# sebadorn/Physically-based-Rendering

Measured on AMD Instinct MI355X. Metric: Msamples/s (paths/s) @1080p fixed seed; 1/2/4/8 MI355X scaling, higher is better.
Workload: dtype f32

## Files before the change

include/pbr_hip_diag.h:

```cpp
#ifndef PBR_HIP_DIAG_H
#define PBR_HIP_DIAG_H

#include "pbr_hip.h"

#ifdef __cplusplus
extern "C" {
#endif

int pbr_diag_math( pbr_ctx* ctx, int op, const float* x, const float* y, int n, float* out );

int pbr_diag_trace( pbr_ctx* ctx, const float* rays, int n, float* out_t, int32_t* out_face, float* out_normal, uint32_t* out_counts );

int pbr_diag_brdf( pbr_ctx* ctx, const float* in, int n, float* out );

int pbr_diag_new_ray( pbr_ctx* ctx, const float* in, int n, float* out );

int pbr_diag_trace_stream( pbr_ctx* ctx, int lds_slots, const float* rays8, uint32_t n, int repeats, float* out2, double* ms_out );

int pbr_diag_calibrate( pbr_ctx* ctx, int mode, uint64_t table_bytes, uint64_t reads, double* ms_out );

int pbr_diag_last_plan( pbr_ctx* ctx, char* name, size_t capacity, int* tuned );

int pbr_diag_bvh_build_info( pbr_ctx* ctx, int* radius );

int pbr_diag_scene_bytes( pbr_ctx* ctx, uint64_t out[3] );

int pbr_diag_refit_info( pbr_ctx* ctx, uint64_t out[8], double* upload_ms, char* why, size_t capacity );

int pbr_diag_last_kernel( pbr_ctx* ctx, char* name, size_t capacity );

int pbr_diag_launch_fit( pbr_ctx* ctx, double* fixed_ms, double* per_frame_ms );

int pbr_diag_set_knob( pbr_ctx* ctx, const char* name, int value );

int pbr_diag_pin_plan( pbr_ctx* ctx, int plan );

int pbr_diag_get_tile_order( pbr_ctx* ctx, int which, uint32_t* order, uint32_t capacity, uint32_t* count, uint32_t band_first[9] );
int pbr_diag_set_tile_order( pbr_ctx* ctx, const uint32_t* order, uint32_t count, const uint32_t* band_first );

int pbr_diag_last_deal( pbr_ctx* ctx, char* name, size_t capacity, int* learnt );
// ... 18 lines not shown
```

physically-based-rendering_amd/__init__.py:

```python
import ctypes
import os

import numpy as np

from . import build as _build
from . import tiles

_HERE = os.path.dirname(os.path.abspath(__file__))

PBR_OK = 0


class Float4(ctypes.Structure):
    _fields_ = [("x", ctypes.c_float), ("y", ctypes.c_float), ("z", ctypes.c_float), ("w", ctypes.c_float)]


class Camera(ctypes.Structure):
    _fields_ = [("eye", Float4), ("w", Float4), ("u", Float4), ("v", Float4),
                ("focusPoint", ctypes.c_int32 * 2), ("lense", ctypes.c_float * 2)]


class DenoiseParams(ctypes.Structure):
    _fields_ = [("passes", ctypes.c_uint32), ("sigma_color", ctypes.c_float), ("sigma_normal", ctypes.c_float),
                ("sigma_world", ctypes.c_float), ("sigma_albedo", ctypes.c_float)]
# ... 110 lines not shown
        ("pbr_mode_built", [ctypes.c_uint32, ctypes.c_uint32]),
        ("pbr_diag_last_kernel", [_vp, ctypes.c_char_p, ctypes.c_size_t]),
        ("pbr_diag_launch_fit", [_vp, ctypes.POINTER(ctypes.c_double), ctypes.POINTER(ctypes.c_double)]),
        ("pbr_diag_set_knob", [_vp, ctypes.c_char_p, ctypes.c_int]),
        ("pbr_diag_get_tile_order", [_vp, ctypes.c_int, _up, ctypes.c_uint32, _up, _up]),
        ("pbr_diag_set_tile_order", [_vp, _up, ctypes.c_uint32, _up]),
        ("pbr_diag_last_deal", [_vp, ctypes.c_char_p, ctypes.c_size_t, ctypes.POINTER(ctypes.c_int)]),
        ("pbr_diag_bvh_build_info", [_vp, ctypes.POINTER(ctypes.c_int)]),
        ("pbr_render_dof", [_vp, ctypes.c_uint32, ctypes.c_uint32, _fp, ctypes.c_float, ctypes.POINTER(Camera)]),
        ("pbr_diag_last_focus_chain", [_vp, ctypes.POINTER(ctypes.c_double)]),
        ("pbr_render_adaptive", [_vp, ctypes.c_uint32, _fp, ctypes.c_float, ctypes.POINTER(Camera), ctypes.POINTER(AdaptiveParams)]),
        ("pbr_read_tile_stats", [_vp, _up, _fp, ctypes.c_uint32, _up]),
        ("pbr_diag_last_adaptive", [_vp, _up, ctypes.POINTER(ctypes.c_uint64), ctypes.POINTER(ctypes.c_double)]),
        ("pbr_update_vertices", [_vp, ctypes.c_void_p, ctypes.c_uint32]),
        ("pbr_read_bvh", [_vp, ctypes.c_void_p, ctypes.c_uint32, _up]),
        ("pbr_diag_refit_info", [_vp, ctypes.POINTER(ctypes.c_uint64), ctypes.POINTER(ctypes.c_double), ctypes.c_char_p, ctypes.c_size_t])):
    if hasattr(hip, _name):
        getattr(hip, _name).argtypes = _args
hip.pbr_diag_tune_budget.argtypes = [_vp, ctypes.POINTER(ctypes.c_uint32)]

host.pbrh_last_error.restype = ctypes.c_char_p
host.pbrh_cfg_set.argtypes = [ctypes.c_char_p, ctypes.c_char_p]
host.pbrh_cfg_get.argtypes = [ctypes.c_char_p, ctypes.c_char_p, ctypes.c_int]
host.pbrh_cfg_load.argtypes = [ctypes.c_char_p]
host.pbrh_scene_load_obj.argtypes = [ctypes.c_char_p, ctypes.c_char_p]
host.pbrh_scene_load_obj.restype = _vp
host.pbrh_scene_generate.argtypes = [ctypes.c_char_p, ctypes.c_uint32, ctypes.c_uint32]
host.pbrh_scene_generate.restype = _vp
host.pbrh_scene_destroy.argtypes = [_vp]
host.pbrh_scene_destroy.restype = None
host.pbrh_scene_desc.argtypes = [_vp, ctypes.POINTER(SceneDesc)]
# ... 359 lines not shown
    def last_trace(self):
        ms, n = ctypes.c_double(), ctypes.c_uint32()
        self._check(hip.pbr_diag_last_trace(self._ctx, ctypes.byref(ms), ctypes.byref(n)))
        return float(ms.value), int(n.value)

    def last_focus_chain_ms(self):
        ms = ctypes.c_double()
        self._check(hip.pbr_diag_last_focus_chain(self._ctx, ctypes.byref(ms)))
        return float(ms.value)

    def last_plan(self):
        name, tuned = ctypes.create_string_buffer(48), ctypes.c_int(-1)
        self._check(hip.pbr_diag_last_plan(self._ctx, name, 48, ctypes.byref(tuned)))
        return name.value.decode(), int(tuned.value)

    def scene_bytes(self):
        out = (ctypes.c_uint64 * 3)()
        self._check(hip.pbr_diag_scene_bytes(self._ctx, out))
        return {"nodes": int(out[0]), "walk_streams": int(out[1]), "faces": int(out[2])}

    def last_kernel(self):
        name = ctypes.create_string_buffer(96)
        self._check(hip.pbr_diag_last_kernel(self._ctx, name, 96))
        return name.value.decode()

    def launch_fit(self):
        a, b = ctypes.c_double(), ctypes.c_double()
        if hip.pbr_diag_launch_fit(self._ctx, ctypes.byref(a), ctypes.byref(b)) != PBR_OK:
            return None
        return float(a.value), float(b.value)
# ... 125 lines not shown
```

physically-based-rendering_amd/csrc/pbr_hip.hip:

```cpp
#include <hip/hip_runtime.h>

#include <cmath>
#include <cstdarg>
#include <cstdio>
#include <cstdlib>
#include <chrono>
#include <cstring>
#include <string>
#include <algorithm>
#include <vector>

#include "pbr_hip.h"
#include "pbr_hip_diag.h"
#include "pt_aux.hpp"
#include "pt_adaptive.hpp"
#include "pt_instances.hpp"
#include "bvh_build.hpp"
#include "pt_denoise.hpp"
#include "pt_scene_pack.hpp"
#include "pt_tuner.hpp"
#include "pt_deal.hpp"
#include "pt_adaptive_host.hpp"
#include "pt_refit_host.hpp"
#include "pt_refit.hpp"
// ... 438 lines not shown
	return PBR_OK;
}

int sceneParams( pbr_ctx* ctx, DevParams* P, uint32_t* hotAvail = nullptr ) {
	std::memset( P, 0, sizeof( *P ) );
	uint32_t hot = 0;
	const int walk = applyWalk( ctx, P, &hot );

	if( hotAvail != nullptr ) {
		*hotAvail = hot;
	}

	P->parkEighths = 4;
	P->tris = ctx->dTris;
	P->faceN = ctx->dFaceN;
	P->mats = ctx->dMats;
	P->lights = ctx->dLights;
	P->guard = ctx->dGuard;
	P->numNodes = (int) ctx->numNodes;
	P->numLights = (int) ctx->numLights;
	return walk;
}

void setCamera( DevParams* P, const pbr_camera* cam, int w, int h, float pxDim ) {
	const float* src[4] = { &cam->eye.x, &cam->w.x, &cam->u.x, &cam->v.x };
	float* dst[4] = { P->eye, P->cw, P->cu, P->cv };

	for( int i = 0; i < 4; i++ ) {
		for( int k = 0; k < 3; k++ ) {
			dst[i][k] = src[i][k];
// ... 741 lines not shown

	if( ctx->configured ) {
		PBR_TRY( packConfiguredWalk( ctx, ctx->cfg, &tree, &walk ) );
	}

	HIP_TRY( ctx, hipSetDevice( ctx->device ) );
	freeScene( ctx );

	auto toDevice = [ctx]( float4** dst, const std::vector<Quad>& src ) {
		HIP_TRY( ctx, hipMalloc( (void**) dst, sizeof( Quad ) * src.size() ) );
		HIP_TRY( ctx, hipMemcpy( *dst, src.data(), sizeof( Quad ) * src.size(), hipMemcpyHostToDevice ) );
		return PBR_OK;
	};

	PBR_TRY( toDevice( &ctx->dNodes, packed.nodes.storage ) );
	PBR_TRY( toDevice( &ctx->dTris, packed.tris ) );

	if( !packed.triPN.empty() ) {
		PBR_TRY( toDevice( &ctx->dTriPN, packed.triPN ) );
	}

	PBR_TRY( toDevice( &ctx->dMats, packed.mats ) );
	PBR_TRY( toDevice( &ctx->dLights, packed.lights ) );
	ctx->nodeBytes = sizeof( Quad ) * packed.nodes.storage.size();
	ctx->triBytes = sizeof( Quad ) * packed.tris.size();

	if( s->num_faces > 0 && ctx->knobs.faceNormals != 0 ) {
		HIP_TRY( ctx, hipMalloc( (void**) &ctx->dFaceN, sizeof( float4 ) * s->num_faces ) );
		DevParams P;
		std::memset( &P, 0, sizeof( P ) );
		P.tris = ctx->dTris;
		hipLaunchKernelGGL( ptk::prepareFaceNormals, dim3( ( s->num_faces + 255 ) / 256 ), dim3( 256 ), 0, ctx->stream, P, ctx->dFaceN, (int) s->num_faces );
		HIP_TRY( ctx, hipGetLastError() );
	}

	ctx->refitBytes = 0;

	if( refit.nested ) {
		auto keep = [ctx]( void** dst, const void* src, size_t bytes ) {
			HIP_TRY( ctx, hipMalloc( dst, std::max<size_t>( bytes, 16 ) ) );

			if( src != nullptr && bytes > 0 ) {
				HIP_TRY( ctx, hipMemcpy( *dst, src, bytes, hipMemcpyHostToDevice ) );
			}

			ctx->refitBytes += bytes;
			return PBR_OK;
		};
// ... 53 lines not shown
	}
	if( ctx->configured && ctx->cfg.phong_tessellation > 0.0f ) {
		return fail( ctx, PBR_ESTATE, "pbr_update_vertices while Phong tessellation is configured: tight boxes of the flat triangles would clip the patches" );
	}

	HIP_TRY( ctx, hipSetDevice( ctx->device ) );
	const auto uploadStart = std::chrono::steady_clock::now();
	HIP_TRY( ctx, hipMemcpy( ctx->dVertices, vertices, sizeof( pbr_float4 ) * num_vertices, hipMemcpyHostToDevice ) );
	ctx->lastRefitUploadMs = std::chrono::duration<double, std::milli>( std::chrono::steady_clock::now() - uploadStart ).count();

	const uint32_t F = ctx->numFaces;
	HIP_TRY( ctx, hipEventRecord( ctx->evStart, ctx->stream ) );
	hipLaunchKernelGGL( ptr::refitFaces, dim3( ( F + 255 ) / 256 ), dim3( 256 ), 0, ctx->stream, ctx->dFacesV, ctx->dVertices, ctx->dTris, (int) F );
	HIP_TRY( ctx, hipGetLastError() );

	if( ctx->dFaceN != nullptr ) {
		DevParams P;
		std::memset( &P, 0, sizeof( P ) );
		P.tris = ctx->dTris;
		hipLaunchKernelGGL( ptk::prepareFaceNormals, dim3( ( F + 255 ) / 256 ), dim3( 256 ), 0, ctx->stream, P, ctx->dFaceN, (int) F );
		HIP_TRY( ctx, hipGetLastError() );
	}

	hipLaunchKernelGGL( ptr::refitSubtrees, dim3( ctx->refitGroups ), dim3( REFIT_SUBTREE ), 0, ctx->stream, ctx->dRefitSlots, ctx->dRefitInfo,
	                    ctx->dRefitHeights, ctx->dRefitRecordOf, ctx->dFacesV, ctx->dVertices, ctx->dNodes, ctx->dRootBox );
	HIP_TRY( ctx, hipGetLastError() );

	if( ctx->refitLevels > 0 ) {
		hipLaunchKernelGGL( ptr::refitTop, dim3( 1 ), dim3( REFIT_TOP_THREADS ), 0, ctx->stream, ctx->dRefitTop, ctx->dRefitLevelFirst, (int) ctx->refitLevels,
		                    ctx->dRefitInfo, ctx->dRefitRecordOf, ctx->dNodes, ctx->dRootBox );
		HIP_TRY( ctx, hipGetLastError() );
	}

	HIP_TRY( ctx, hipEventRecord( ctx->evStop, ctx->stream ) );
	HIP_TRY( ctx, hipStreamSynchronize( ctx->stream ) );
	float ms = 0.0f;
// ... 980 lines not shown
	*radius = ctx->lastBvhRadius;
	return PBR_OK;
}

int pbr_diag_scene_bytes( pbr_ctx* ctx, uint64_t out[3] ) {
	if( ctx == nullptr || out == nullptr || !ctx->hasScene ) {
		return fail( ctx, PBR_ESTATE, "diag_scene_bytes: no scene" );
	}

	out[0] = ctx->nodeBytes;
	out[1] = ctx->walkBytes;
	out[2] = ctx->triBytes;
	return PBR_OK;
}

int pbr_diag_refit_info( pbr_ctx* ctx, uint64_t out[8], double* upload_ms, char* why, size_t capacity ) {
	if( ctx == nullptr || out == nullptr || !ctx->hasScene ) {
		return fail( ctx, PBR_ESTATE, "diag_refit_info: no scene" );
	}

	out[0] = ctx->refit.nested ? 1 : 0;
	out[1] = ctx->refit.subtreeCap;
	out[2] = ctx->refitGroups;
	out[3] = ctx->refitSubtrees;
	out[4] = ctx->refitTopNodes;
	out[5] = ctx->refitLevels;
	out[6] = ctx->refitBytes;
	out[7] = ctx->refitUpdates;

	if( upload_ms != nullptr ) {
// ... 179 lines not shown
```

physically-based-rendering_amd/csrc/pt_aux.hpp:

```cpp
#pragma once

#include "pt_kernel.hpp"
#include "pt_diag.hpp"

namespace ptk {

__global__ __launch_bounds__( 256 ) void foldFrames( const DevParams P, const float4* src, float4* dst ) {
	const unsigned slot = blockIdx.x * blockDim.x + threadIdx.x;

	if( slot <= (unsigned) PT_HEADS ) {
		P.workCounter[slot * PT_BAND_STRIDE] = 0u;
	}

	if( slot >= P.frameStride ) {
		return;
	}

	float4 acc = src[slot];

	for( int k = 0; k < P.nFrames; k++ ) {
		const float4 fc = P.frameBuf[frameBufIndex( P, slot, (unsigned) k )];
		const unsigned n = (unsigned) ( P.firstCount + k );
		const float w = P.useExplicitWeight ? P.explicitWeight : ( (float) n / (float) ( n + 1u ) );
		acc.x = fc.x + ( acc.x - fc.x ) * w;
// ... 21 lines not shown
	if( ( threadIdx.x & 63u ) == 0u ) {
		cost[tile] = v;
	}
}

__global__ void prepareFaceNormals( DevParams P, float4* faceN, int numFaces ) {
	const int face = (int) ( blockIdx.x * blockDim.x + threadIdx.x );

	if( face >= numFaces ) {
		return;
	}

	int material;
	const f3 n = faceNormal<false>( P, face, &material );
	faceN[face] = make_float4( n.x, n.y, n.z, __int_as_float( material ) );
}


__global__ void untile( const float4* tiles, float4* rows, int width, int height, int tilesX, int tileWorld, int tileRank ) {
	const int x = (int) ( blockIdx.x * blockDim.x + threadIdx.x );
	const int y = (int) ( blockIdx.y * blockDim.y + threadIdx.y );

	if( x >= width || y >= height ) {
		return;
	}

	const int tileGlobal = ( y >> 3 ) * tilesX + ( x >> 3 );
	float4 v = make_float4( 0.0f, 0.0f, 0.0f, 0.0f );

	const int position = dealPositionOfTile( tileGlobal, tilesX, tileWorld );
// ... 173 lines not shown
```

physically-based-rendering_amd/csrc/pt_dual.hpp:

```cpp
#ifdef PT_NODE_PHASE_ASM

#define PT_DUAL_SLAB( n0a, n0b, n0c, n0d, n1a, n1b, oxy, ozz, ixy, izz ) \
		"v_pk_add_f32 v[54:55], v[" n0a ":" n0b "], " oxy " neg_lo:[0,1] neg_hi:[0,1]\n" \
		"v_pk_add_f32 v[56:57], v[" n0c ":" n0d "], " oxy " neg_lo:[0,1] neg_hi:[0,1]\n" \
		"v_pk_add_f32 v[58:59], v[" n1a ":" n1b "], " ozz " neg_lo:[0,1] neg_hi:[0,1]\n" \
		"v_pk_mul_f32 v[54:55], " ixy ", v[54:55]\n" \
		"v_pk_mul_f32 v[56:57], " ixy ", v[56:57]\n" \
		"v_pk_mul_f32 v[58:59], " izz ", v[58:59]\n" \
		"v_min_f32 v60, v54, v56\n" \
		"v_min_f32 v61, v55, v57\n" \
		"v_min_f32 v62, v58, v59\n" \
		"v_max3_f32 v60, v60, v61, v62\n" \
		"v_max_f32 v61, v54, v56\n" \
		"v_max_f32 v63, v58, v59\n" \
		"v_max_f32 v62, v55, v57\n" \
		"v_min3_f32 v61, v61, v62, v63\n"
#define PT_DUAL_FETCH( walk, cur, n0, n1lo, n1hi, flag, skip ) \
		"s_mov_b64 exec, " walk "\n" \
		"s_cbranch_execz " skip "9f\n" \
		"v_cmp_gt_i32 vcc, %[numHotBytes], " cur "\n" \
		"s_and_saveexec_b64 s[94:95], vcc\n" \
		"s_cselect_b32 s82, 1, 0\n" \
		"ds_read_b128 v[" n0 "], " cur "\n" \
		"ds_read_b128 v[" n1lo ":" n1hi "], " cur " offset:16\n" \
// ... 282 lines not shown
			if( ( shadeA || shadeB ) && ( nShade >= P.phShade || !busy ) ) {
				const bool useB = !shadeA;
				const int which = useB ? 1 : 0;
				PixelState st;
				loadCold( P, which, st );
				st.ray.origin = useB ? B.ray.origin : A.ray.origin;
				st.ray.dir = useB ? B.ray.dir : A.ray.dir;
				st.dbgNodes += useB ? B.nodes : A.nodes;
				st.dbgTris += useB ? B.tris : A.tris;
				Hit hit;
				hit.t = useB ? B.t : A.t;
				hit.face = useB ? B.face : A.face;
				hit.normal = mk3( 0.0f, 0.0f, 0.0f );
				bool more = true;

				if( shadeStep<BRDF, SHADOW, LIGHTS, false, true, true>( P, lds, st, cnt, hit ) ) {
					finishPixel( P, st );

					if( cnt.nodes > 0x40000000u || cnt.tris > 0x40000000u ) {
						flushCounters( P, cnt );
					}

					unsigned frame = 0;
					const unsigned slot = nextSlot( P, work, (unsigned) P.nFrames, frame );

					if( slot != PT_NO_WORK ) {
						beginPixel( P, st, slot, cnt, frame );
					}
					else {
						more = false;
					}
// ... 20 lines not shown
```

physically-based-rendering_amd/csrc/pt_kernel.hpp:

```cpp
#pragma once

#include <hip/hip_runtime.h>

#include "pt_math.hpp"

#ifdef PBR_GUARD
#define PBR_GUARD_PATH 1
#define PBR_GUARD_TRAV 1
#endif

#ifdef PBR_LAB_HOOKS
#include "pt_lab_hooks.hpp"
#else
#define PT_LAB_TRAVERSE_BEGIN
#define PT_LAB_NODE_ITERATION
#define PT_LAB_LEAF_PHASE
#define PT_LAB_TRAVERSE_END( P, anyhit )
#define PT_LAB_WAVE_BEGIN
#define PT_LAB_WAVE_DRY
#define PT_LAB_WAVE_END_LOCKSTEP( P )
#define PT_LAB_WAVE_END_PHASED( P )
#define PT_LAB_PHASED_BEGIN
#define PT_LAB_PHASED_STAT( what )
#define PT_LAB_PHASED_NODE_BEGIN( mode )
// ... 76 lines not shown
	int numHot;
	int numHotBytes;
	int firstRef;
	int walkScheme;
	const int* walkTable;
	int slotBase;
	int nFrames, firstCount;
	int useExplicitWeight;
	float explicitWeight;
	float pxDim, antiAliasing;
	float sky[3];
	const float4* faceN;
	const float* chain;
	unsigned chainSlotStride, chainFrameStride;
	unsigned chainFocusAt;
};

#define PT_DEAL_SHIFT 5

__host__ __device__ inline int dealPositionOfTile( int tileGlobal, int tilesX, int world ) {
	if( world <= 1 ) {
		return tileGlobal;
	}

	const int ty = tileGlobal / tilesX;
	const int tx = tileGlobal - ty * tilesX;
	return ty * tilesX + ( tx + PT_DEAL_SHIFT * ty ) % tilesX;
}

__host__ __device__ inline int tileAtDealPosition( int position, int tilesX, int world ) {
// ... 32 lines not shown
PT_DEV f3 ld3( const float* p ) { return mk3( p[0], p[1], p[2] ); }

PT_DEV float rnd( float& seed ) {
	seed += 1.0f;
	return fract( sin1( seed ) * 43758.5453123f );
}

PT_DEV float fresnel( float u, float c ) {
	const float v = 1.0f - u;
	return c + ( 1.0f - c ) * v * v * v * v * v;
}

struct TangentFrame {
	f3 n, u, v;
	bool valid;
};

PT_DEV void tangentFrame( f3 n, f3* u, f3* v ) {
	*u = normalize( cross( yzx( n ), n ) );
	*v = normalize( cross( n, *u ) );
}

PT_DEV bool sameBits( f3 a, f3 b ) {
	return __float_as_int( a.x ) == __float_as_int( b.x ) && __float_as_int( a.y ) == __float_as_int( b.y ) && __float_as_int( a.z ) == __float_as_int( b.z );
}

PT_DEV f3 jitterUV( f3 nl, f3 u, f3 v, float phi, float sina, float cosa ) {
	float sp, cp;
	sincos( phi, &sp, &cp );
	const f3 w = normalize( u * cp + v * sp );
	return normalize( w * sina + nl * cosa );
}

PT_DEV f3 jitter( f3 nl, float phi, float sina, float cosa ) {
	f3 u, v;
	tangentFrame( nl, &u, &v );
	return jitterUV( nl, u, v, phi, sina, cosa );
}

// ... 3 lines not shown
	const float4 b = P.mats[index * 4 + 1];
	Material m;
	m.d = a.x; m.Ni = a.y; m.p2 = a.z; m.p3 = a.w;
	m.Rs = b.x; m.Rd = b.y;
	m.colours = P.mats + index * 4 + 2;
	m.Kd = m.Ks = mk3( 0.0f, 0.0f, 0.0f );

	if( !LATE ) {
		const float4 kd = m.colours[0];
		const float4 ks = m.colours[1];
		m.Kd = mk3( kd.x, kd.y, kd.z );
		m.Ks = mk3( ks.x, ks.y, ks.z );
	}

	return m;
}

template<bool LATE = true>
PT_DEV MaterialColours materialColours( const Material& m ) {
	MaterialColours c;

	if( LATE ) {
		const float4 kd = m.colours[0];
		const float4 ks = m.colours[1];
		c.Kd = mk3( kd.x, kd.y, kd.z );
		c.Ks = mk3( ks.x, ks.y, ks.z );
	}
	else {
		c.Kd = m.Kd;
		c.Ks = m.Ks;
// ... 857 lines not shown
PT_DEV f3 faceNormal( const DevParams& P, int face, int* material ) {
	if( STORED && !PT_ARITH_NATIVE && P.faceN != nullptr ) {
		const float4 r = P.faceN[face];
		*material = __float_as_int( r.w );
		return mk3( r.x, r.y, r.z );
	}

	const float4 r0 = P.tris[face * 3 + 0];
	const float4 r1 = P.tris[face * 3 + 1];
	const float4 r2 = P.tris[face * 3 + 2];
	*material = __float_as_int( r2.y );
	return normalize( cross( mk3( r0.w, r1.x, r1.y ), mk3( r1.z, r1.w, r2.x ) ) );
}



PT_DEV Ray initRay( const DevParams& P, int px, int py, float& seed, float tFocus, float tObject ) {
	const f3 cu = ld3( P.cu );
	const f3 cv = ld3( P.cv );
	const float fx = 2.0f * (float) px;
	const float fy = 2.0f * (float) py;

	f3 inner = ld3( P.camA );
	inner = inner + cu * fx;
	inner = inner + cv;
	inner = inner - ld3( P.cvH );
	inner = inner + cv * fy;

	const float s = P.halfPx;
	const f3 initial = ld3( P.cw ) + inner * s;
// ... 41 lines not shown
	return ( x == 0.0f ) ? 0.0f : div1( r, x * x );
}

PT_DEV float schA( float w, float p ) {
	const float p2 = p * p;
	const float w2 = w * w;
	const float x = p2 - p2 * w2 + w2;
	return ( x == 0.0f ) ? 0.0f : sqrt1( div1( p, x ) );
}

PT_DEV float schG( float v, float r ) {
	const float x = r - r * v + v;
	return ( x == 0.0f ) ? 0.0f : div1( v, x );
}

PT_DEV float brdfSchlick( const Material& mtl, f3 outDir, f3 inDir, f3 normal, float* u, float* pdf, const TangentFrame* frame = nullptr ) {
	const f3 vOutV = -outDir;
	f3 un;

	if( frame != nullptr && frame->valid && sameBits( frame->n, normal ) ) {
		un = frame->u;
	}
	else {
		un = normalize( cross( yzx( normal ), normal ) );
	}

	const f3 h = normalize( vOutV + inDir );
	const float t = dot( h, normal );
	const float vIn = dot( inDir, normal );
	const float vOut = dot( vOutV, normal );
	const f3 hp = normalize( cross( cross( h, normal ), normal ) );
	const float w = dot( un, hp );

	*u = dot( h, vOutV );
	*pdf = div1( t, (float) ( (double) 4.0f * M_PI_D * (double) dot( vOutV, h ) ) );
// ... 7 lines not shown
	const float lam = (float) ( (double) a * M_1_PI_D );
	float ani = 0.0f;

	if( !( b == 0.0f || d == 0.0f ) ) {
		const float gp = schG( vOut, r ) * schG( vIn, r );
		const float obstructed = gp * schZ( t, r ) * schA( w, p );
		const float reemission = 1.0f - gp;
		ani = div1( b, d ) * ( obstructed + reemission );
	}

	const float fres = ( vIn == 0.0f ) ? 0.0f : div1( c, vIn );

	return lam + ani + fres;
}

PT_DEV f3 newRaySchlick( f3 dir, f3 normal, const Material& mtl, float& seed, TangentFrame* frame = nullptr ) {
	const float rough = mtl.p3;
	const float iso = mtl.p2;

	if( rough == 0.0f ) {
		return reflect( dir, normal );
	}

	const float a = rnd( seed );
	float b = rnd( seed );
	const float iso2 = iso * iso;
	const float alpha = acos1( sqrt1( div1( a, rough - a * rough + a ) ) );
	float edge, base;
	int mode;

// ... 7 lines not shown
	base = (float) ( M_PI_2_D * (double) sqrt1( div1( iso2 * b2, 1.0f - b2 + b2 * iso2 ) ) );

	float phi = base;

	if( mode == 1 ) { phi = (float) ( M_PI_D - (double) base ); }
	else if( mode == 2 ) { phi = (float) ( M_PI_D + (double) base ); }
	else if( mode == 3 ) { phi = (float) ( (double) 2.0f * M_PI_D - (double) base ); }

	if( iso < 1.0f ) {
		phi = (float) ( (double) phi + M_PI_2_D );
	}

	float sa, ca;
	sincos( alpha, &sa, &ca );
	f3 fu, fv;
	tangentFrame( normal, &fu, &fv );

	if( frame != nullptr ) {
		frame->n = normal;
		frame->u = fu;
		frame->v = fv;
		frame->valid = true;
	}

	const f3 H = jitterUV( normal, fu, fv, phi, sa, ca );
	f3 out = reflect( dir, H );

	if( dot( out, normal ) <= 0.0f ) {
		out = jitterUV( normal, fu, fv, PI_X2 * rnd( seed ), sqrt1( a ), sqrt1( 1.0f - a ) );
	}

	return out;
}



template<bool CALLS = false>
PT_DEV void brdfSA(
	const Material& mtl, f3 outDir, f3 inDir, f3 normal,
	float* brdfSpec, float* brdfDiff, float* dotHK1, float* pdf, const TangentFrame* frame = nullptr
) {
	const float nu = mtl.p2, nv = mtl.p3;
	f3 un, vn;

	if( frame != nullptr && frame->valid && sameBits( frame->n, normal ) ) {
		un = frame->u;
		vn = frame->v;
	}
	else {
		tangentFrame( normal, &un, &vn );
	}

	const f3 k1 = inDir;
	const f3 k2 = -outDir;
	const f3 h = normalize( k1 + k2 );

	const float dotHU = dot( h, un );
	const float dotHV = dot( h, vn );
	const float dotHN = dot( h, normal );
	const float dotNK1 = dot( normal, k1 );
	const float dotNK2 = dot( normal, k2 );
	const float hk1 = dot( h, k1 );
	*dotHK1 = hk1;

	float ps_e = nu * dotHU * dotHU + nv * dotHV * dotHV;
	ps_e = ( dotHN == 1.0f ) ? 0.0f : div1( ps_e, 1.0f - dotHN * dotHN );
	const float ps0 = (float) ( (double) ( sqrt1( ( nu + 1.0f ) * ( nv + 1.0f ) ) * 0.125f ) * M_1_PI_D );
	const float ps1_num = powSelect<CALLS>( dotHN, ps_e );
	const float ps1 = div1( ps1_num, hk1 * fmax1( dotNK1, dotNK2 ) );

	float pd = mtl.Rd * 0.38750768752f;
	const float a = 1.0f - dotNK1 * 0.5f;
	const float b = 1.0f - dotNK2 * 0.5f;
	pd *= 1.0f - a * a * a * a * a;
	pd *= 1.0f - b * b * b * b * b;

	*brdfSpec = ps0 * ps1;
	*brdfDiff = pd;
	*pdf = div1( ps0 * ps1_num, hk1 );
}

template<bool CALLS = false>
PT_DEV f3 newRaySA( f3 dir, f3 rayNormal, const Material& mtl, float& seed, TangentFrame* frame = nullptr ) {
	const float nu = mtl.p2, nv = mtl.p3;
	float a = rnd( seed );
	const float b = rnd( seed );
	float phi_flip = (float) M_PI_D;
	float phi_flipf = 1.0f;
	float aMax = 1.0f;

	if( a < 0.25f ) {
		aMax = 0.25f;
		phi_flip = 0.0f;
	}
	else if( a < 0.5f ) {
		aMax = 0.5f;
		phi_flipf = -1.0f;
	}
	else if( a < 0.75f ) {
		aMax = 0.75f;
	}
	else {
		phi_flip = (float) ( (double) 2.0f * M_PI_D );
		phi_flipf = -1.0f;
	}

	a = 1.0f - 4.0f * ( aMax - a );

	const float phi = atan1( sqrt1( div1( nu + 1.0f, nv + 1.0f ) ) * tan1( (float) ( M_PI_2_D * (double) a ) ) );
	const float phi_full = phi_flip + phi_flipf * phi;

	float sinphi, cosphi;
	sincos( phi, &sinphi, &cosphi );
	const float theta_e = div1( 1.0f, nu * cosphi * cosphi + nv * sinphi * sinphi + 1.0f );
	const float theta = acos1( powSelect<CALLS>( 1.0f - b, theta_e ) );

	const f3 normal = ( mtl.d < 1.0f || dot( rayNormal, -dir ) >= 0.0f ) ? rayNormal : -rayNormal;

	float st, ct;
	sincos( theta, &st, &ct );
	f3 u, v;
	tangentFrame( normal, &u, &v );

	if( frame != nullptr ) {
		frame->n = normal;
		frame->u = u;
		frame->v = v;
		frame->valid = true;
	}

	const f3 h = jitterUV( normal, u, v, phi_full, st, ct );
	const f3 spec = reflect( dir, h );
	const f3 diff = jitterUV( normal, u, v, PI_X2 * rnd( seed ), sqrt1( b ), sqrt1( 1.0f - b ) );

	return ( dot( spec, normal ) <= 0.0f ) ? diff : spec;
}

PT_DEV f3 refract( f3 dir, f3 normal, const Material& mtl, float& seed ) {
	const bool into = ( dot( normal, -dir ) > 0.0f );
	const f3 nl = into ? normal : -normal;
	const float m1 = into ? NI_AIR : mtl.Ni;
	const float m2 = into ? mtl.Ni : NI_AIR;
	const float m = div1( m1, m2 );
// ... 5 lines not shown
	}

	const float sqrtCosT = sqrt1( 1.0f - sinT2 );
	const float r0 = div1( m1 - m2, m1 + m2 );
	const float c = ( m1 > m2 ) ? sqrtCosT : cosI;
	const float reflectance = fresnel( c, r0 * r0 );

	if( reflectance < rnd( seed ) ) {
		const float k = m * cosI - sqrtCosT;
		return dir * m + nl * k;
	}

	return reflect( dir, nl );
}

template<int BRDF, bool CALLS = false>
PT_DEV f3 newRayDir( f3 dir, f3 normal, const Material& mtl, float& seed, bool& addDepth, TangentFrame* frame = nullptr ) {
	bool doTransRefr = false;

	if( mtl.d < 1.0f ) {
		doTransRefr = ( mtl.d <= rnd( seed ) );
	}

	addDepth = addDepth || doTransRefr;

	if( doTransRefr ) {
		return refract( dir, normal, mtl, seed );
	}

	return ( BRDF == 0 ) ? newRaySchlick( dir, normal, mtl, seed, frame ) : newRaySA<CALLS>( dir, normal, mtl, seed, frame );
}

template<int BRDF, bool CALLS = false, bool LATE = true>
PT_DEV f3 throughput( const Material& mtl, f3 outDir, f3 inDir, f3 normal, const TangentFrame* frame = nullptr ) {
	const float d = mtl.d;

	if( BRDF == 0 ) {
		float u, pdf;
		float brdf = brdfSchlick( mtl, outDir, inDir, normal, &u, &pdf, frame );
		brdf *= fmax1( dot( normal, inDir ), 0.0f );
		brdf = div1( brdf, pdf );

		const MaterialColours mc = materialColours<LATE>( mtl );
		const f3 f4 = mk3( fresnel( u, mc.Ks.x ), fresnel( u, mc.Ks.y ), fresnel( u, mc.Ks.z ) );
		const f3 k = mk3( f4.x * brdf * d + ( 1.0f - d ), f4.y * brdf * d + ( 1.0f - d ), f4.z * brdf * d + ( 1.0f - d ) );
		return mc.Kd * k;
	}

	float spec, diff, dotHK1, pdf;
	brdfSA<CALLS>( mtl, outDir, inDir, normal, &spec, &diff, &dotHK1, &pdf, frame );
	spec = div1( spec, pdf );
	diff = div1( diff, pdf );

	const float fr = fresnel( dotHK1, mtl.Rs );
	const MaterialColours mc = materialColours<LATE>( mtl );
	const f3 brdf_s = ( mc.Ks * spec ) * fr;
	const f3 brdf_d = ( mc.Kd * diff ) * ( 1.0f - mtl.Rs );
	f3 bc = brdf_s + brdf_d;
	bc = mk3( bc.x * d + ( 1.0f - d ), bc.y * d + ( 1.0f - d ), bc.z * d + ( 1.0f - d ) );
	const float maxRGB = max_cl( 1.0f, max_cl( bc.x, max_cl( bc.y, bc.z ) ) );
	bc = mk3( div1( bc.x, maxRGB ), div1( bc.y, maxRGB ), div1( bc.z, maxRGB ) );

	return mk3( clamp01( bc.x ), clamp01( bc.y ), clamp01( bc.z ) );
}

template<int BRDF, bool CALLS = false, bool LATE = true>
PT_DEV bool shadowContribution(
	const Material& mtl, f3 outDir, f3 lightDir, f3 normal, f3 color, f3 lightRgb, f3* add, const TangentFrame* frame = nullptr
) {
	const float d = mtl.d;

	if( BRDF == 0 ) {
		float u, pdf;
		float brdf = brdfSchlick( mtl, outDir, lightDir, normal, &u, &pdf, frame );

		if( !( __builtin_fabsf( pdf ) > 0.00001f ) ) {
			return false;
		}

		brdf *= fmax1( dot( normal, lightDir ), 0.0f );
		brdf = div1( brdf, pdf );

		const MaterialColours mc = materialColours<LATE>( mtl );
		const f3 f4 = mk3( fresnel( u, mc.Ks.x ), fresnel( u, mc.Ks.y ), fresnel( u, mc.Ks.z ) );
		const f3 k = mk3( f4.x * brdf * d + ( 1.0f - d ), f4.y * brdf * d + ( 1.0f - d ), f4.z * brdf * d + ( 1.0f - d ) );
		*add = ( ( color * lightRgb ) * mc.Kd ) * k;
		return true;
	}

	float spec, diff, dotHK1, pdf;
	brdfSA<CALLS>( mtl, outDir, lightDir, normal, &spec, &diff, &dotHK1, &pdf, frame );

	if( !( __builtin_fabsf( pdf ) > 0.00001f ) ) {
		return false;
	}

	spec = div1( spec, pdf );
	diff = div1( diff, pdf );

	const float fr = fresnel( dotHK1, mtl.Rs );
	const MaterialColours mc = materialColours<LATE>( mtl );
	const f3 brdf_s = ( mc.Ks * spec ) * fr;
	const f3 brdf_d = ( mc.Kd * diff ) * ( 1.0f - mtl.Rs );
	f3 bc = brdf_s + brdf_d;
	bc = mk3( bc.x * d + ( 1.0f - d ), bc.y * d + ( 1.0f - d ), bc.z * d + ( 1.0f - d ) );
	const float maxRGB = max_cl( 1.0f, max_cl( bc.x, max_cl( bc.y, bc.z ) ) );
// ... 108 lines not shown
	st.depthAdded = 0;
	float tFocus, tObject;
	focusInputs( P, slot, frame, &tFocus, &tObject );
	int px, py;
	pixelOfSlot( P, slot, &px, &py );
	st.ray = initRay( P, px, py, st.seed, tFocus, tObject );
	cnt.paths++;
}

PT_DEV void finishPixel( const DevParams& P, const PixelState& st ) {
	if( P.imgDbg != nullptr && st.frame == P.nFrames ) {
		P.imgDbg[st.slot] = make_float4( (float) st.dbgTris / 1082.0f, (float) st.dbgNodes / 1265.0f, 0.0f, 0.0f );
	}
}

template<int BRDF, bool SHADOW, bool LIGHTS, bool PHONG = false, bool EAGER = false, bool CALLS = !EAGER, bool FACEN = false, bool LATE = true>
PT_DEV bool shadeStep( const DevParams& P, const float4* lds, PixelState& st, LaneCounters& cnt, const Hit hit ) {
	Ray& ray = st.ray;
	f3& color = st.color;
	f3& finalColor = st.finalColor;
	unsigned& secondaryPaths = st.secondaryPaths;
	float& seed = st.seed;
	int& depth = st.depth;
	int& depthAdded = st.depthAdded;
	unsigned& dbgTris = st.dbgTris;
	unsigned& totHits = cnt.hits;

	st.focus = ( st.sample + depth == 0 ) ? hit.t : st.focus;

		bool pathDone = false;
		f3 light = mk3( -1.0f, -1.0f, -1.0f );

		if( hit.t == inff() ) {
			if( LIGHTS && hit.face < 0 ) {
				const float4 rgb = P.lights[( -( hit.face + 1 ) ) * 3 + 1];
				light = mk3( rgb.x, rgb.y, rgb.z );
			}
			else {
				light = ld3( P.sky );
			}

			pathDone = true;
		}
		else {
			int mtlIndex;
			f3 normal = faceNormal<FACEN>( P, hit.face, &mtlIndex );

			if( PHONG ) {
				normal = hit.normal;
			}
			const Material mtl = loadMaterial<LATE>( P, mtlIndex );
			totHits++;

			bool addDepth;

			if( BRDF == 1 ) {
				addDepth = ( fmax1( mtl.p2, mtl.p3 ) >= 50.0f );
			}
			else {
				addDepth = ( mtl.p3 < rnd( seed ) );
			}
// ... 24 lines not shown
						lh.face = 0;
						unsigned unusedNodes = 0;
						traverse<true, LIGHTS, true, PHONG, EAGER>( P, lds, lightRay, lh, unusedNodes, dbgTris );
						lightDir = lightRay.dir;

						if( lh.t >= tLight ) {
							const float4 rgb = P.lights[1];
							lightRgb = mk3( rgb.x, rgb.y, rgb.z );
							lit = ( lightRgb.x >= 0.0f );
						}
					}
				}

				TangentFrame frame;
				frame.valid = false;
				const f3 newDir = newRayDir<BRDF, CALLS>( ray.dir, normal, mtl, seed, addDepth, &frame );

				if( dot( normal, -ray.dir ) <= 0.0f ) {
					normal = -normal;
				}

				if( SHADOW && LIGHTS ) {
					if( lit ) {
						f3 add;

						if( shadowContribution<BRDF, CALLS, LATE>( mtl, ray.dir, lightDir, normal, color, lightRgb, &add, &frame ) ) {
							finalColor = finalColor + add;
							secondaryPaths += 1;
						}
					}
				}

				color = color * throughput<BRDF, CALLS, LATE>( mtl, ray.dir, newDir, normal, &frame );

				depthAdded += ( addDepth && depthAdded < P.maxAddedDepth ) ? 1 : 0;

				const float maxValColor = fmax1( color.x, fmax1( color.y, color.z ) );
				bool terminate = false;

				if( depth > 2 + depthAdded ) {
					terminate = ( maxValColor < rnd( seed ) );
				}

				if( terminate ) {
					pathDone = true;
				}
				else {
					ray.origin = hitPoint;
// ... 401 lines not shown
```

physically-based-rendering_amd/csrc/pt_scene_pack.hpp:

```cpp
#pragma once

#include <algorithm>
#include <cmath>
#include <cstdarg>
#include <cstddef>
#include <cstdint>
#include <cstdio>
#include <cstring>
#include <string>
#include <utility>
#include <vector>

#include "pbr_hip.h"

struct Quad {
	float x, y, z, w;
};
static_assert( sizeof( Quad ) == 16, "a Quad is a float4 on the device" );

constexpr uint32_t kLdsStageBytes = 160 * 1024 - 256;

constexpr size_t kRefLimit = (size_t) 1 << 31;

struct SceneTree {
// ... 488 lines not shown
		}
	}

	const uint32_t lightSlots = ( s->num_lights > 0 ) ? s->num_lights : 1;
	out->lights.assign( (size_t) lightSlots * 3, Quad { 0.0f, 0.0f, 0.0f, 0.0f } );

	for( uint32_t i = 0; i < s->num_lights; i++ ) {
		const pbr_light& l = s->lights[i];
		out->lights[(size_t) i * 3 + 0] = Quad { l.pos.x, l.pos.y, l.pos.z, l.pos.w };
		out->lights[(size_t) i * 3 + 1] = Quad { l.rgb.x, l.rgb.y, l.rgb.z, l.rgb.w };
		out->lights[(size_t) i * 3 + 2] = Quad { l.data.x, l.data.y, l.data.z, l.data.w };
	}

	return PBR_OK;
}
```

Before: 2242.

## Precompute per-face tangent frames and per-material BRDF terms on device

Adds a scene-load and refit pass that stores, for each face, its normal, material index, tangent frame and the tangent frame of the flipped normal, appended after the triangle data. The shading path loads these records instead of rebuilding the frame at every hit. Per-material Ashikhmin-Shirley constants (ps0 and the phi scale) are also packed into the material table so the sqrt/div work per bounce goes away. The cost is extra memory traffic per hit (up to three more float4 loads) and a larger triangle buffer, with a fallback to on-the-fly computation when a stored frame is flagged non-bitwise-identical.

```diff
diff --git a/include/pbr_hip_diag.h b/include/pbr_hip_diag.h
--- a/include/pbr_hip_diag.h
+++ b/include/pbr_hip_diag.h
@@ -24,6 +24,8 @@
 int pbr_diag_bvh_build_info( pbr_ctx* ctx, int* radius );
 
 int pbr_diag_scene_bytes( pbr_ctx* ctx, uint64_t out[3] );
+
+int pbr_diag_face_frames( pbr_ctx* ctx, float* records, float* per_hit );
 
 int pbr_diag_refit_info( pbr_ctx* ctx, uint64_t out[8], double* upload_ms, char* why, size_t capacity );
 
diff --git a/physically-based-rendering_amd/__init__.py b/physically-based-rendering_amd/__init__.py
--- a/physically-based-rendering_amd/__init__.py
+++ b/physically-based-rendering_amd/__init__.py
@@ -148,7 +148,8 @@
         ("pbr_diag_last_adaptive", [_vp, _up, ctypes.POINTER(ctypes.c_uint64), ctypes.POINTER(ctypes.c_double)]),
         ("pbr_update_vertices", [_vp, ctypes.c_void_p, ctypes.c_uint32]),
         ("pbr_read_bvh", [_vp, ctypes.c_void_p, ctypes.c_uint32, _up]),
-        ("pbr_diag_refit_info", [_vp, ctypes.POINTER(ctypes.c_uint64), ctypes.POINTER(ctypes.c_double), ctypes.c_char_p, ctypes.c_size_t])):
+        ("pbr_diag_refit_info", [_vp, ctypes.POINTER(ctypes.c_uint64), ctypes.POINTER(ctypes.c_double), ctypes.c_char_p, ctypes.c_size_t]),
+        ("pbr_diag_face_frames", [_vp, _fp, _fp])):
     if hasattr(hip, _name):
         getattr(hip, _name).argtypes = _args
 hip.pbr_diag_tune_budget.argtypes = [_vp, ctypes.POINTER(ctypes.c_uint32)]
@@ -538,6 +539,12 @@
         self._check(hip.pbr_diag_last_plan(self._ctx, name, 48, ctypes.byref(tuned)))
         return name.value.decode(), int(tuned.value)
 
+    def diag_face_frames(self, num_faces):
+        records = np.empty((num_faces, 16), np.float32)
+        per_hit = np.empty((num_faces, 16), np.float32)
+        self._check(hip.pbr_diag_face_frames(self._ctx, _as_fp(records), _as_fp(per_hit)))
+        return records.view(np.uint32), per_hit.view(np.uint32)
+
     def scene_bytes(self):
         out = (ctypes.c_uint64 * 3)()
         self._check(hip.pbr_diag_scene_bytes(self._ctx, out))
diff --git a/physically-based-rendering_amd/csrc/pbr_hip.hip b/physically-based-rendering_amd/csrc/pbr_hip.hip
--- a/physically-based-rendering_amd/csrc/pbr_hip.hip
+++ b/physically-based-rendering_amd/csrc/pbr_hip.hip
@@ -476,6 +476,7 @@
 	P->parkEighths = 4;
 	P->tris = ctx->dTris;
 	P->faceN = ctx->dFaceN;
+	P->frameFirst = (int) frameFirstQuad( ctx->numFaces );
 	P->mats = ctx->dMats;
 	P->lights = ctx->dLights;
 	P->guard = ctx->dGuard;
@@ -1247,24 +1248,32 @@
 	};
 
 	PBR_TRY( toDevice( &ctx->dNodes, packed.nodes.storage ) );
-	PBR_TRY( toDevice( &ctx->dTris, packed.tris ) );
+	HIP_TRY( ctx, hipMalloc( (void**) &ctx->dTris, sizeof( Quad ) * faceAllocationQuads( s->num_faces ) ) );
+	HIP_TRY( ctx, hipMemset( ctx->dTris, 0, sizeof( Quad ) * faceAllocationQuads( s->num_faces ) ) );
+	HIP_TRY( ctx, hipMemcpy( ctx->dTris, packed.tris.data(), sizeof( Quad ) * packed.tris.size(), hipMemcpyHostToDevice ) );
 
 	if( !packed.triPN.empty() ) {
 		PBR_TRY( toDevice( &ctx->dTriPN, packed.triPN ) );
 	}
 
+	packMaterialTerms( s, &packed.mats );
 	PBR_TRY( toDevice( &ctx->dMats, packed.mats ) );
 	PBR_TRY( toDevice( &ctx->dLights, packed.lights ) );
 	ctx->nodeBytes = sizeof( Quad ) * packed.nodes.storage.size();
-	ctx->triBytes = sizeof( Quad ) * packed.tris.size();
-
-	if( s->num_faces > 0 && ctx->knobs.faceNormals != 0 ) {
-		HIP_TRY( ctx, hipMalloc( (void**) &ctx->dFaceN, sizeof( float4 ) * s->num_faces ) );
+	ctx->triBytes = sizeof( Quad ) * faceAllocationQuads( s->num_faces );
+
+	{
 		DevParams P;
 		std::memset( &P, 0, sizeof( P ) );
 		P.tris = ctx->dTris;
-		hipLaunchKernelGGL( ptk::prepareFaceNormals, dim3( ( s->num_faces + 255 ) / 256 ), dim3( 256 ), 0, ctx->stream, P, ctx->dFaceN, (int) s->num_faces );
+		hipLaunchKernelGGL( ptk::prepareFaceFrames, dim3( ( s->num_faces + 255 ) / 256 ), dim3( 256 ), 0, ctx->stream, P, ctx->dTris + frameFirstQuad( s->num_faces ), (int) s->num_faces );
 		HIP_TRY( ctx, hipGetLastError() );
+
+		if( ctx->knobs.faceNormals != 0 ) {
+			HIP_TRY( ctx, hipMalloc( (void**) &ctx->dFaceN, sizeof( float4 ) * s->num_faces ) );
+			hipLaunchKernelGGL( ptk::prepareFaceNormals, dim3( ( s->num_faces + 255 ) / 256 ), dim3( 256 ), 0, ctx->stream, P, ctx->dFaceN, (int) s->num_faces );
+			HIP_TRY( ctx, hipGetLastError() );
+		}
 	}
 
 	ctx->refitBytes = 0;
@@ -1348,12 +1357,17 @@
 	hipLaunchKernelGGL( ptr::refitFaces, dim3( ( F + 255 ) / 256 ), dim3( 256 ), 0, ctx->stream, ctx->dFacesV, ctx->dVertices, ctx->dTris, (int) F );
 	HIP_TRY( ctx, hipGetLastError() );
 
-	if( ctx->dFaceN != nullptr ) {
+	{
 		DevParams P;
 		std::memset( &P, 0, sizeof( P ) );
 		P.tris = ctx->dTris;
-		hipLaunchKernelGGL( ptk::prepareFaceNormals, dim3( ( F + 255 ) / 256 ), dim3( 256 ), 0, ctx->stream, P, ctx->dFaceN, (int) F );
+		hipLaunchKernelGGL( ptk::prepareFaceFrames, dim3( ( F + 255 ) / 256 ), dim3( 256 ), 0, ctx->stream, P, ctx->dTris + frameFirstQuad( F ), (int) F );
 		HIP_TRY( ctx, hipGetLastError() );
+
+		if( ctx->dFaceN != nullptr ) {
+			hipLaunchKernelGGL( ptk::prepareFaceNormals, dim3( ( F + 255 ) / 256 ), dim3( 256 ), 0, ctx->stream, P, ctx->dFaceN, (int) F );
+			HIP_TRY( ctx, hipGetLastError() );
+		}
 	}
 
 	hipLaunchKernelGGL( ptr::refitSubtrees, dim3( ctx->refitGroups ), dim3( REFIT_SUBTREE ), 0, ctx->stream, ctx->dRefitSlots, ctx->dRefitInfo,
@@ -2364,6 +2378,40 @@
 	return PBR_OK;
 }
 
+int pbr_diag_face_frames( pbr_ctx* ctx, float* records, float* per_hit ) {
+	if( ctx == nullptr || records == nullptr || per_hit == nullptr ) {
+		return fail( ctx, PBR_EINVAL, "diag_face_frames: null argument" );
+	}
+	if( !ctx->hasScene ) {
+		return fail( ctx, PBR_ESTATE, "diag_face_frames: no scene" );
+	}
+
+	const uint32_t F = ctx->numFaces;
+	const size_t bytes = sizeof( float ) * 16 * (size_t) F;
+	float* dOut = nullptr;
+	HIP_TRY( ctx, hipSetDevice( ctx->device ) );
+	HIP_TRY( ctx, hipMalloc( (void**) &dOut, bytes ) );
+	DevParams P;
+	std::memset( &P, 0, sizeof( P ) );
+	P.tris = ctx->dTris;
+	hipLaunchKernelGGL( ptk::faceFramesPerHit, dim3( ( F + 255 ) / 256 ), dim3( 256 ), 0, ctx->stream, P, dOut, (int) F );
+	hipError_t err = hipGetLastError();
+
+	if( err == hipSuccess ) {
+		err = hipStreamSynchronize( ctx->stream );
+	}
+	if( err == hipSuccess ) {
+		err = hipMemcpy( per_hit, dOut, bytes, hipMemcpyDeviceToHost );
+	}
+	if( err == hipSuccess ) {
+		err = hipMemcpy( records, ctx->dTris + frameFirstQuad( F ), bytes, hipMemcpyDeviceToHost );
+	}
+
+	(void) hipFree( dOut );
+	HIP_TRY( ctx, err );
+	return PBR_OK;
+}
+
 int pbr_diag_refit_info( pbr_ctx* ctx, uint64_t out[8], double* upload_ms, char* why, size_t capacity ) {
 	if( ctx == nullptr || out == nullptr || !ctx->hasScene ) {
 		return fail( ctx, PBR_ESTATE, "diag_refit_info: no scene" );
diff --git a/physically-based-rendering_amd/csrc/pt_aux.hpp b/physically-based-rendering_amd/csrc/pt_aux.hpp
--- a/physically-based-rendering_amd/csrc/pt_aux.hpp
+++ b/physically-based-rendering_amd/csrc/pt_aux.hpp
@@ -59,6 +59,49 @@
 	int material;
 	const f3 n = faceNormal<false>( P, face, &material );
 	faceN[face] = make_float4( n.x, n.y, n.z, __int_as_float( material ) );
+}
+
+__global__ void prepareFaceFrames( DevParams P, float4* frames, int numFaces ) {
+	const int face = (int) ( blockIdx.x * blockDim.x + threadIdx.x );
+
+	if( face >= numFaces ) {
+		return;
+	}
+
+	int material;
+	const f3 n = faceNormal<false>( P, face, &material );
+	f3 u, v, ub, vb;
+	tangentFrame( n, &u, &v );
+	tangentFrame( -n, &ub, &vb );
+	const float sum = ( ( n.x + n.y + n.z ) + ( u.x + u.y + u.z ) ) + ( ( v.x + v.y + v.z ) + ( vb.x + vb.y + vb.z ) );
+	const bool finite = ( __builtin_fabsf( sum ) < inff() );
+	const int flags = ( finite && sameBits( u, ub ) ) ? 0 : 1;
+	float4* rec = frames + (size_t) face * PT_FRAME_QUADS;
+	rec[0] = make_float4( n.x, n.y, n.z, __int_as_float( material ) );
+	rec[1] = make_float4( u.x, u.y, u.z, __int_as_float( flags ) );
+	rec[2] = make_float4( v.x, v.y, v.z, 0.0f );
+	rec[3] = make_float4( vb.x, vb.y, vb.z, 0.0f );
+}
+
+__global__ void faceFramesPerHit( DevParams P, float* out, int numFaces ) {
+	const int face = (int) ( blockIdx.x * blockDim.x + threadIdx.x );
+
+	if( face >= numFaces ) {
+		return;
+	}
+
+	int material;
+	const f3 n = faceNormal<false>( P, face, &material );
+	f3 u, v, ub, vb;
+	tangentFrame( n, &u, &v );
+	tangentFrame( -n, &ub, &vb );
+	float* o = out + (size_t) face * 16;
+	o[0] = n.x; o[1] = n.y; o[2] = n.z;
+	o[3] = u.x; o[4] = u.y; o[5] = u.z;
+	o[6] = v.x; o[7] = v.y; o[8] = v.z;
+	o[9] = ub.x; o[10] = ub.y; o[11] = ub.z;
+	o[12] = vb.x; o[13] = vb.y; o[14] = vb.z;
+	o[15] = __int_as_float( material );
 }
 
 
diff --git a/physically-based-rendering_amd/csrc/pt_dual.hpp b/physically-based-rendering_amd/csrc/pt_dual.hpp
--- a/physically-based-rendering_amd/csrc/pt_dual.hpp
+++ b/physically-based-rendering_amd/csrc/pt_dual.hpp
@@ -320,7 +320,9 @@
 				hit.normal = mk3( 0.0f, 0.0f, 0.0f );
 				bool more = true;
 
-				if( shadeStep<BRDF, SHADOW, LIGHTS, false, true, true>( P, lds, st, cnt, hit ) ) {
+				constexpr bool FRAMES = !( PT_WALK_MODE == 1 && BRDF == 1 && SHADOW );
+
+				if( shadeStep<BRDF, SHADOW, LIGHTS, false, true, true, false, true, FRAMES>( P, lds, st, cnt, hit ) ) {
 					finishPixel( P, st );
 
 					if( cnt.nodes > 0x40000000u || cnt.tris > 0x40000000u ) {
diff --git a/physically-based-rendering_amd/csrc/pt_kernel.hpp b/physically-based-rendering_amd/csrc/pt_kernel.hpp
--- a/physically-based-rendering_amd/csrc/pt_kernel.hpp
+++ b/physically-based-rendering_amd/csrc/pt_kernel.hpp
@@ -114,6 +114,7 @@
 	const float* chain;
 	unsigned chainSlotStride, chainFrameStride;
 	unsigned chainFocusAt;
+	int frameFirst;
 };
 
 #define PT_DEAL_SHIFT 5
@@ -176,6 +177,9 @@
 struct TangentFrame {
 	f3 n, u, v;
 	bool valid;
+	bool flipped;
+	const float4* tris;
+	int record;
 };
 
 PT_DEV void tangentFrame( f3 n, f3* u, f3* v ) {
@@ -185,6 +189,27 @@
 
 PT_DEV bool sameBits( f3 a, f3 b ) {
 	return __float_as_int( a.x ) == __float_as_int( b.x ) && __float_as_int( a.y ) == __float_as_int( b.y ) && __float_as_int( a.z ) == __float_as_int( b.z );
+}
+
+#ifndef PT_FACE_FRAMES
+#define PT_FACE_FRAMES 1
+#endif
+#ifndef PT_MATERIAL_TERMS
+#define PT_MATERIAL_TERMS 1
+#endif
+#define PT_FRAME_QUADS 4
+
+PT_DEV bool storedFrame( const TangentFrame* frame, bool negated, f3* u, f3* v ) {
+	const float4 q1 = frame->tris[frame->record + 1];
+
+	if( __float_as_int( q1.w ) != 0 ) {
+		return false;
+	}
+
+	const float4 q2 = frame->tris[frame->record + ( negated ? 3 : 2 )];
+	*u = mk3( q1.x, q1.y, q1.z );
+	*v = mk3( q2.x, q2.y, q2.z );
+	return true;
 }
 
 PT_DEV f3 jitterUV( f3 nl, f3 u, f3 v, float phi, float sina, float cosa ) {
@@ -218,6 +243,11 @@
 	}
 
 	return m;
+}
+
+PT_DEV float materialTerm( const Material& m, int which ) {
+	const float4 b = m.colours[-1];
+	return ( which == 0 ) ? b.z : b.w;
 }
 
 template<bool LATE = true>
@@ -1105,6 +1135,12 @@
 }
 
 
+PT_DEV f3 frameNormal( const DevParams& P, int face, int* material ) {
+	const float4 q0 = P.tris[P.frameFirst + face * PT_FRAME_QUADS];
+	*material = __float_as_int( q0.w );
+	return mk3( q0.x, q0.y, q0.z );
+}
+
 
 PT_DEV Ray initRay( const DevParams& P, int px, int py, float& seed, float tFocus, float tObject ) {
 	const f3 cu = ld3( P.cu );
@@ -1176,11 +1212,20 @@
 	return ( x == 0.0f ) ? 0.0f : div1( v, x );
 }
 
+template<bool STORED = false>
 PT_DEV float brdfSchlick( const Material& mtl, f3 outDir, f3 inDir, f3 normal, float* u, float* pdf, const TangentFrame* frame = nullptr ) {
 	const f3 vOutV = -outDir;
 	f3 un;
 
-	if( frame != nullptr && frame->valid && sameBits( frame->n, normal ) ) {
+
+	if constexpr( STORED && PT_FACE_FRAMES ) {
+		f3 vn;
+
+		if( !storedFrame( frame, frame->flipped, &un, &vn ) ) {
+			un = normalize( cross( yzx( normal ), normal ) );
+		}
+	}
+	else if( frame != nullptr && frame->valid && sameBits( frame->n, normal ) ) {
 		un = frame->u;
 	}
 	else {
@@ -1218,6 +1263,7 @@
 	return lam + ani + fres;
 }
 
+template<bool STORED = false>
 PT_DEV f3 newRaySchlick( f3 dir, f3 normal, const Material& mtl, float& seed, TangentFrame* frame = nullptr ) {
 	const float rough = mtl.p3;
 	const float iso = mtl.p2;
@@ -1255,13 +1301,21 @@
 	float sa, ca;
 	sincos( alpha, &sa, &ca );
 	f3 fu, fv;
-	tangentFrame( normal, &fu, &fv );
-
-	if( frame != nullptr ) {
-		frame->n = normal;
-		frame->u = fu;
-		frame->v = fv;
-		frame->valid = true;
+
+	if constexpr( STORED && PT_FACE_FRAMES ) {
+		if( !storedFrame( frame, false, &fu, &fv ) ) {
+			tangentFrame( normal, &fu, &fv );
+		}
+	}
+	else {
+		tangentFrame( normal, &fu, &fv );
+
+		if( frame != nullptr ) {
+			frame->n = normal;
+			frame->u = fu;
+			frame->v = fv;
+			frame->valid = true;
+		}
 	}
 
 	const f3 H = jitterUV( normal, fu, fv, phi, sa, ca );
@@ -1276,7 +1330,7 @@
 
 
 
-template<bool CALLS = false>
+template<bool CALLS = false, bool STORED = false>
 PT_DEV void brdfSA(
 	const Material& mtl, f3 outDir, f3 inDir, f3 normal,
 	float* brdfSpec, float* brdfDiff, float* dotHK1, float* pdf, const TangentFrame* frame = nullptr
@@ -1284,7 +1338,12 @@
 	const float nu = mtl.p2, nv = mtl.p3;
 	f3 un, vn;
 
-	if( frame != nullptr && frame->valid && sameBits( frame->n, normal ) ) {
+	if constexpr( STORED && PT_FACE_FRAMES ) {
+		if( !storedFrame( frame, frame->flipped, &un, &vn ) ) {
+			tangentFrame( normal, &un, &vn );
+		}
+	}
+	else if( frame != nullptr && frame->valid && sameBits( frame->n, normal ) ) {
 		un = frame->u;
 		vn = frame->v;
 	}
@@ -1306,7 +1365,7 @@
 
 	float ps_e = nu * dotHU * dotHU + nv * dotHV * dotHV;
 	ps_e = ( dotHN == 1.0f ) ? 0.0f : div1( ps_e, 1.0f - dotHN * dotHN );
-	const float ps0 = (float) ( (double) ( sqrt1( ( nu + 1.0f ) * ( nv + 1.0f ) ) * 0.125f ) * M_1_PI_D );
+	const float ps0 = ( STORED && PT_MATERIAL_TERMS ) ? materialTerm( mtl, 0 ) : (float) ( (double) ( sqrt1( ( nu + 1.0f ) * ( nv + 1.0f ) ) * 0.125f ) * M_1_PI_D );
 	const float ps1_num = powSelect<CALLS>( dotHN, ps_e );
 	const float ps1 = div1( ps1_num, hk1 * fmax1( dotNK1, dotNK2 ) );
 
@@ -1321,7 +1380,7 @@
 	*pdf = div1( ps0 * ps1_num, hk1 );
 }
 
-template<bool CALLS = false>
+template<bool CALLS = false, bool STORED = false>
 PT_DEV f3 newRaySA( f3 dir, f3 rayNormal, const Material& mtl, float& seed, TangentFrame* frame = nullptr ) {
 	const float nu = mtl.p2, nv = mtl.p3;
 	float a = rnd( seed );
@@ -1348,7 +1407,15 @@
 
 	a = 1.0f - 4.0f * ( aMax - a );
 
-	const float phi = atan1( sqrt1( div1( nu + 1.0f, nv + 1.0f ) ) * tan1( (float) ( M_PI_2_D * (double) a ) ) );
+	float phi;
+
+	if constexpr( STORED && PT_MATERIAL_TERMS ) {
+		phi = atan1( materialTerm( mtl, 1 ) * tan1( (float) ( M_PI_2_D * (double) a ) ) );
+	}
+	else {
+		phi = atan1( sqrt1( div1( nu + 1.0f, nv + 1.0f ) ) * tan1( (float) ( M_PI_2_D * (double) a ) ) );
+	}
+
 	const float phi_full = phi_flip + phi_flipf * phi;
 
 	float sinphi, cosphi;
@@ -1361,13 +1428,21 @@
 	float st, ct;
 	sincos( theta, &st, &ct );
 	f3 u, v;
-	tangentFrame( normal, &u, &v );
-
-	if( frame != nullptr ) {
-		frame->n = normal;
-		frame->u = u;
-		frame->v = v;
-		frame->valid = true;
+
+	if constexpr( STORED && PT_FACE_FRAMES ) {
+		if( !storedFrame( frame, __float_as_int( normal.x ) != __float_as_int( rayNormal.x ), &u, &v ) ) {
+			tangentFrame( normal, &u, &v );
+		}
+	}
+	else {
+		tangentFrame( normal, &u, &v );
+
+		if( frame != nullptr ) {
+			frame->n = normal;
+			frame->u = u;
+			frame->v = v;
+			frame->valid = true;
+		}
 	}
 
 	const f3 h = jitterUV( normal, u, v, phi_full, st, ct );
@@ -1403,7 +1478,7 @@
 	return reflect( dir, nl );
 }
 
-template<int BRDF, bool CALLS = false>
+template<int BRDF, bool CALLS = false, bool STORED = false>
 PT_DEV f3 newRayDir( f3 dir, f3 normal, const Material& mtl, float& seed, bool& addDepth, TangentFrame* frame = nullptr ) {
 	bool doTransRefr = false;
 
@@ -1417,16 +1492,16 @@
 		return refract( dir, normal, mtl, seed );
 	}
 
-	return ( BRDF == 0 ) ? newRaySchlick( dir, normal, mtl, seed, frame ) : newRaySA<CALLS>( dir, normal, mtl, seed, frame );
-}
-
-template<int BRDF, bool CALLS = false, bool LATE = true>
+	return ( BRDF == 0 ) ? newRaySchlick<STORED>( dir, normal, mtl, seed, frame ) : newRaySA<CALLS, STORED>( dir, normal, mtl, seed, frame );
+}
+
+template<int BRDF, bool CALLS = false, bool LATE = true, bool STORED = false>
 PT_DEV f3 throughput( const Material& mtl, f3 outDir, f3 inDir, f3 normal, const TangentFrame* frame = nullptr ) {
 	const float d = mtl.d;
 
 	if( BRDF == 0 ) {
 		float u, pdf;
-		float brdf = brdfSchlick( mtl, outDir, inDir, normal, &u, &pdf, frame );
+		float brdf = brdfSchlick<STORED>( mtl, outDir, inDir, normal, &u, &pdf, frame );
 		brdf *= fmax1( dot( normal, inDir ), 0.0f );
 		brdf = div1( brdf, pdf );
 
@@ -1437,7 +1512,7 @@
 	}
 
 	float spec, diff, dotHK1, pdf;
-	brdfSA<CALLS>( mtl, outDir, inDir, normal, &spec, &diff, &dotHK1, &pdf, frame );
+	brdfSA<CALLS, STORED>( mtl, outDir, inDir, normal, &spec, &diff, &dotHK1, &pdf, frame );
 	spec = div1( spec, pdf );
 	diff = div1( diff, pdf );
 
@@ -1453,7 +1528,7 @@
 	return mk3( clamp01( bc.x ), clamp01( bc.y ), clamp01( bc.z ) );
 }
 
-template<int BRDF, bool CALLS = false, bool LATE = true>
+template<int BRDF, bool CALLS = false, bool LATE = true, bool STORED = false>
 PT_DEV bool shadowContribution(
 	const Material& mtl, f3 outDir, f3 lightDir, f3 normal, f3 color, f3 lightRgb, f3* add, const TangentFrame* frame = nullptr
 ) {
@@ -1461,7 +1536,7 @@
 
 	if( BRDF == 0 ) {
 		float u, pdf;
-		float brdf = brdfSchlick( mtl, outDir, lightDir, normal, &u, &pdf, frame );
+		float brdf = brdfSchlick<STORED>( mtl, outDir, lightDir, normal, &u, &pdf, frame );
 
 		if( !( __builtin_fabsf( pdf ) > 0.00001f ) ) {
 			return false;
@@ -1478,7 +1553,7 @@
 	}
 
 	float spec, diff, dotHK1, pdf;
-	brdfSA<CALLS>( mtl, outDir, lightDir, normal, &spec, &diff, &dotHK1, &pdf, frame );
+	brdfSA<CALLS, STORED>( mtl, outDir, lightDir, normal, &spec, &diff, &dotHK1, &pdf, frame );
 
 	if( !( __builtin_fabsf( pdf ) > 0.00001f ) ) {
 		return false;
@@ -1617,7 +1692,7 @@
 	}
 }
 
-template<int BRDF, bool SHADOW, bool LIGHTS, bool PHONG = false, bool EAGER = false, bool CALLS = !EAGER, bool FACEN = false, bool LATE = true>
+template<int BRDF, bool SHADOW, bool LIGHTS, bool PHONG = false, bool EAGER = false, bool CALLS = !EAGER, bool FACEN = false, bool LATE = true, bool FRAMES = false>
 PT_DEV bool shadeStep( const DevParams& P, const float4* lds, PixelState& st, LaneCounters& cnt, const Hit hit ) {
 	Ray& ray = st.ray;
 	f3& color = st.color;
@@ -1647,7 +1722,8 @@
 		}
 		else {
 			int mtlIndex;
-			f3 normal = faceNormal<FACEN>( P, hit.face, &mtlIndex );
+			constexpr bool STORED = FRAMES && !PHONG && !PT_ARITH_NATIVE;
+			f3 normal = ( STORED && PT_FACE_FRAMES ) ? frameNormal( P, hit.face, &mtlIndex ) : faceNormal<FACEN>( P, hit.face, &mtlIndex );
 
 			if( PHONG ) {
 				normal = hit.normal;
@@ -1702,24 +1778,28 @@
 
 				TangentFrame frame;
 				frame.valid = false;
-				const f3 newDir = newRayDir<BRDF, CALLS>( ray.dir, normal, mtl, seed, addDepth, &frame );
+				frame.flipped = false;
+				frame.tris = P.tris;
+				frame.record = P.frameFirst + hit.face * PT_FRAME_QUADS;
+				const f3 newDir = newRayDir<BRDF, CALLS, STORED>( ray.dir, normal, mtl, seed, addDepth, &frame );
 
 				if( dot( normal, -ray.dir ) <= 0.0f ) {
 					normal = -normal;
+					frame.flipped = true;
 				}
 
 				if( SHADOW && LIGHTS ) {
 					if( lit ) {
 						f3 add;
 
-						if( shadowContribution<BRDF, CALLS, LATE>( mtl, ray.dir, lightDir, normal, color, lightRgb, &add, &frame ) ) {
+						if( shadowContribution<BRDF, CALLS, LATE, STORED>( mtl, ray.dir, lightDir, normal, color, lightRgb, &add, &frame ) ) {
 							finalColor = finalColor + add;
 							secondaryPaths += 1;
 						}
 					}
 				}
 
-				color = color * throughput<BRDF, CALLS, LATE>( mtl, ray.dir, newDir, normal, &frame );
+				color = color * throughput<BRDF, CALLS, LATE, STORED>( mtl, ray.dir, newDir, normal, &frame );
 
 				depthAdded += ( addDepth && depthAdded < P.maxAddedDepth ) ? 1 : 0;
 
diff --git a/physically-based-rendering_amd/csrc/pt_scene_pack.hpp b/physically-based-rendering_amd/csrc/pt_scene_pack.hpp
--- a/physically-based-rendering_amd/csrc/pt_scene_pack.hpp
+++ b/physically-based-rendering_amd/csrc/pt_scene_pack.hpp
@@ -526,3 +526,34 @@
 
 	return PBR_OK;
 }
+
+inline void materialTerms( float nu, float nv, float* ps0, float* phiK ) {
+	const float a = nu + 1.0f, b = nv + 1.0f;
+	const float prod = a * b;
+	const float quot = a / b;
+	const float eighth = std::sqrt( prod ) * 0.125f;
+	*ps0 = (float) ( (double) eighth * 0x1.45f306dc9c883p-2 );
+	*phiK = std::sqrt( quot );
+}
+
+inline void packMaterialTerms( const pbr_scene_desc* s, std::vector<Quad>* mats ) {
+	if( s->brdf != 1 ) {
+		return;
+	}
+
+	for( uint32_t i = 0; i < s->num_materials; i++ ) {
+		const Quad& a = ( *mats )[(size_t) i * 4 + 0];
+		Quad& b = ( *mats )[(size_t) i * 4 + 1];
+		materialTerms( a.z, a.w, &b.z, &b.w );
+	}
+}
+
+constexpr size_t kFrameQuads = 4;
+
+inline size_t frameFirstQuad( size_t numFaces ) {
+	return ( ( numFaces + 1 ) * 3 + 3 ) / 4 * 4;
+}
+
+inline size_t faceAllocationQuads( size_t numFaces ) {
+	return frameFirstQuad( numFaces ) + numFaces * kFrameQuads;
+}
```

New measurement: 2211. 0.986x the previous value.
